# aerius-labs/paillier-halo2

Measured on AMD Instinct MI355X. Metric: Paillier-encrypt proofs/s (2048-bit n, k=17); MSM achieved HBM GB/s vs peak, higher is better.
Workload: dtype u32 limbs (29-bit reduced radix, 254-bit modular integers), u64 limbs (4096-bit integers)

## Files before the change

### paillier_halo2_amd/csrc/pz_quotient.hip

```cpp
#include "fp29.cuh"
#include "pz_internal.h"

static inline Fr fp_one_host() {
    static const uint64_t ONE[4] = {0xac96341c4ffffffbULL, 0x36fc76959f60cd29ULL, 0x666ea36f7879462eULL, 0x0e0a77c19a07df2fULL};
    Fr r;
    memcpy(r.v, ONE, 32);
    return r;
}
static inline Fr fr_from_u64(const uint64_t x[4]) {
    Fr r;
    memcpy(r.v, x, 32);
    return r;
}

typedef F29<FrTag> Fr29;
__device__ __forceinline__ Fr29 fr29_c261(const Fr& c) { return f29_to_261(f29_from_fp(c)); }
__device__ __forceinline__ Fr29 fr29_one256() {
    Fr29 r;
#pragma unroll
    for (int i = 0; i < 9; ++i) r.v[i] = P29<FrTag>::R256(i);
    return r;
}

struct S29 {
    u32 v[9];
};
static bool host_fr_canonical(const uint64_t c[4]) {
    static const uint64_t R[4] = {0x43e1f593f0000001ULL, 0x2833e84879b97091ULL, 0xb85045b68181585dULL, 0x30644e72e131a029ULL};
    for (int i = 3; i >= 0; --i)
        if (c[i] != R[i]) return c[i] < R[i];
    return false;
}
static S29 host_fr_shl(const uint64_t c[4], unsigned k) {
    static const uint64_t R[4] = {0x43e1f593f0000001ULL, 0x2833e84879b97091ULL, 0xb85045b68181585dULL, 0x30644e72e131a029ULL};
    uint64_t x[4] = {c[0], c[1], c[2], c[3]};
    for (unsigned t = 0; t < k; ++t) {
        for (int i = 3; i > 0; --i) x[i] = (x[i] << 1) | (x[i - 1] >> 63);
        x[0] <<= 1;
        bool ge = true;
        for (int i = 3; i >= 0; --i)
            if (x[i] != R[i]) { ge = x[i] > R[i]; break; }
        if (ge) {
            unsigned __int128 br = 0;
            for (int i = 0; i < 4; ++i) {
                const unsigned __int128 d = (unsigned __int128)x[i] - R[i] - br;
                x[i] = (uint64_t)d;
                br = (d >> 64) & 1;
            }
        }
    }
    S29 r;
    for (int i = 0; i < 9; ++i) {
        const unsigned bit = 29u * i, j = bit >> 6, o = bit & 63;
        uint64_t w = x[j] >> o;
        if (o > 35 && j + 1 < 4) w |= x[j + 1] << (64 - o);
        r.v[i] = (u32)(w & (i < 8 ? 0x1fffffffull : 0xffffffffull));
    }
    return r;
}
static void host_fr_mul(const uint64_t a[4], const uint64_t b[4], uint64_t out[4]) {
    static const uint64_t R[4] = {0x43e1f593f0000001ULL, 0x2833e84879b97091ULL, 0xb85045b68181585dULL, 0x30644e72e131a029ULL};
    const uint64_t INV = 0xc2e1f593efffffffULL;
    uint64_t t[6] = {0, 0, 0, 0, 0, 0};
    for (int i = 0; i < 4; ++i) {
        unsigned __int128 c = 0;
        for (int j = 0; j < 4; ++j) {
            c += (unsigned __int128)a[j] * b[i] + t[j];
            t[j] = (uint64_t)c;
            c >>= 64;
        }
        c += t[4];
        t[4] = (uint64_t)c;
        t[5] = (uint64_t)(c >> 64);
        const uint64_t m = t[0] * INV;
        c = ((unsigned __int128)m * R[0] + t[0]) >> 64;
        for (int j = 1; j < 4; ++j) {
            c += (unsigned __int128)m * R[j] + t[j];
            t[j - 1] = (uint64_t)c;
            c >>= 64;
        }
        c += t[4];
        t[3] = (uint64_t)c;
        t[4] = t[5] + (uint64_t)(c >> 64);
    }
    bool ge = t[4] != 0;
    if (!ge) {
        ge = true;
        for (int i = 3; i >= 0; --i)
            if (t[i] != R[i]) { ge = t[i] > R[i]; break; }
    }
    if (ge) {
        unsigned __int128 br = 0;
        for (int i = 0; i < 4; ++i) {
            const unsigned __int128 d = (unsigned __int128)t[i] - R[i] - br;
            t[i] = (uint64_t)d;
            br = (d >> 64) & 1;
        }
    }
    memcpy(out, t, 32);
}
static void host_fr_pow(const uint64_t a[4], unsigned e, uint64_t out[4]) {
    static const uint64_t ONE[4] = {0xac96341c4ffffffbULL, 0x36fc76959f60cd29ULL, 0x666ea36f7879462eULL, 0x0e0a77c19a07df2fULL};
    uint64_t acc[4], sq[4];
    memcpy(acc, ONE, 32);
    memcpy(sq, a, 32);
    for (; e; e >>= 1) {
        if (e & 1) host_fr_mul(acc, sq, acc);
        host_fr_mul(sq, sq, sq);
    }
    memcpy(out, acc, 32);
}
extern "C" int pzx_host_selftest(void) {
    static const uint64_t ONE[4] = {0xac96341c4ffffffbULL, 0x36fc76959f60cd29ULL, 0x666ea36f7879462eULL, 0x0e0a77c19a07df2fULL};
    auto limbs_of = [](const uint64_t x[4]) { return host_fr_shl(x, 0); };
    auto same = [](const S29& a, const S29& b) { return memcmp(a.v, b.v, sizeof a.v) == 0; };
    uint64_t two[4], acc[4], pw[4];
    {
        const S29 d = host_fr_shl(ONE, 1);
        unsigned __int128 carry = 0;
        memset(two, 0, sizeof two);
        for (int i = 0; i < 9; ++i) {
            const unsigned bit = 29u * i, j = bit >> 6, o = bit & 63;
            two[j] |= (uint64_t)d.v[i] << o;
            if (o > 35 && j + 1 < 4) two[j + 1] |= (uint64_t)d.v[i] >> (64 - o);
        }
        (void)carry;
    }
    if (!same(limbs_of(two), host_fr_shl(ONE, 1))) return 1;
    host_fr_mul(ONE, ONE, acc);
    if (memcmp(acc, ONE, 32)) return 2;
    memcpy(acc, ONE, 32);
    for (unsigned k = 1; k <= 300; ++k) {
        host_fr_mul(acc, two, acc);
        if (!same(limbs_of(acc), host_fr_shl(ONE, k))) return 100 + (int)k;
        if (k % 37 == 0 || k == 300) {
            host_fr_pow(two, k, pw);
            if (memcmp(pw, acc, 32)) return 1000 + (int)k;
        }
    }
    return 0;
}
extern "C" void pzx_host_fr_mul(const uint64_t a[4], const uint64_t b[4], uint64_t out[4]) { host_fr_mul(a, b, out); }
extern "C" void pzx_host_fr_pow(const uint64_t a[4], unsigned e, uint64_t out[4]) { host_fr_pow(a, e, out); }
extern "C" void pzx_host_fr_shl(const uint64_t c[4], unsigned k, uint32_t out[9]) {
    const S29 r = host_fr_shl(c, k);
    memcpy(out, r.v, sizeof r.v);
}
__device__ __forceinline__ Fr29 f29_add_s(const Fr29& a, const u32 (&b)[9]) {
    Fr29 r;
#pragma unroll
    for (int i = 0; i < 9; ++i) r.v[i] = a.v[i] + b[i];
    return r;
}

__global__ __launch_bounds__(256) void k_batch_invert(Fr* __restrict__ a, Fr* __restrict__ scratch, size_t n, size_t T,
                                                      unsigned K, Fr* __restrict__ mul_io) {
    const size_t t = (size_t)blockIdx.x * blockDim.x + threadIdx.x;
    if (t >= T) return;
    Fr29 acc = fr29_one256();
    for (unsigned j = 0; j < K; ++j) {
        const size_t i = t + (size_t)j * T;
        if (i >= n) break;
        const Fr v = fp_load<FrTag>(a + i);
        if (fp_is_zero(v)) continue;
        Fr w;
        f29_pack(acc, w.v);
        fp_store(scratch + i, w);
        acc = f29_mul(acc, f29_from_fp_shl5(v));
    }
    Fr29 inv = f29_mul(f29_inv(acc), fr29_one256());
    for (unsigned j = K; j-- > 0;) {
        const size_t i = t + (size_t)j * T;
        if (i >= n) continue;
        const Fr v = fp_load<FrTag>(a + i);
        if (fp_is_zero(v)) {
            if (mul_io) fp_store(mul_io + i, fp_zero<FrTag>());
            continue;
        }
        const Fr29 ai = f29_mul(inv, f29_load<FrTag>(scratch + i));
        if (mul_io) f29_store_product(mul_io + i, f29_mul(ai, f29_load_shl5<FrTag>(mul_io + i)));
        else f29_store_product(a + i, ai);
        inv = f29_mul(inv, f29_from_fp_shl5(v));
    }
}

int pz_batch_invert_internal(pz_ctx* ctx, Fr* d_a, size_t n, Fr* d_mul_io) {
    if (!n) return PZ_OK;
    void* scr;
    PZCHK(pz_ws_get(ctx, WS_BIG_A, n * 32, &scr));
    unsigned K = 8;
    while (K < 64 && n / (K * 2) >= 16384) K *= 2;
    while (K < 512 && n / (K * 2) >= 262144) K *= 2;
    const size_t T = pz_div_up(n, K);
    hipLaunchKernelGGL(k_batch_invert, dim3(pz_div_up(T, 256)), dim3(256), 0, ctx->stream, d_a, (Fr*)scr, n, T, K, d_mul_io);
    HIPCHK(ctx, hipGetLastError());
    return PZ_OK;
}

extern "C" int pz_fr_batch_invert_dev(pz_ctx* ctx, uint64_t* d_a, size_t n) {
    if (!ctx || (n && !d_a)) return PZ_ERR_INVALID;
    PZ_ENTER(ctx);
    return pz_batch_invert_internal(ctx, (Fr*)d_a, n, nullptr);
}

#define PP_K 16u
__global__ __launch_bounds__(256) void k_pp_local(const Fr* __restrict__ a, size_t as, size_t n, Fr* __restrict__ excl,
                                                  Fr* __restrict__ block_tot, unsigned nb) {
    __shared__ u32 s[9 * 256];
    a += (size_t)blockIdx.y * as;
    const size_t t = (size_t)blockIdx.x * 256 + threadIdx.x;
    const size_t lo = t * PP_K;
    Fr29 p = fr29_one256();
    for (unsigned j = 0; j < PP_K; ++j)
        if (lo + j < n) p = f29_mul(p, f29_load_shl5<FrTag>(a + lo + j));
    p = f29_to_261(p);
#pragma unroll
    for (int i = 0; i < 9; ++i) s[i * 256 + threadIdx.x] = p.v[i];
    __syncthreads();
    for (unsigned off = 1; off < 256; off <<= 1) {
        Fr29 u;
        if (threadIdx.x >= off) {
#pragma unroll
            for (int i = 0; i < 9; ++i) u.v[i] = s[i * 256 + threadIdx.x - off];
        }
        __syncthreads();
        if (threadIdx.x >= off) {
            p = f29_mul(u, p);
#pragma unroll
            for (int i = 0; i < 9; ++i) s[i * 256 + threadIdx.x] = p.v[i];
        }
        __syncthreads();
    }
    Fr29 e = f29_one<FrTag>();
    if (threadIdx.x) {
#pragma unroll
        for (int i = 0; i < 9; ++i) e.v[i] = s[i * 256 + threadIdx.x - 1];
    }
    Fr w;
    f29_pack(e, w.v);
    fp_store(excl + (size_t)blockIdx.y * nb * 256 + t, w);
    if (threadIdx.x == 255) f29_store_product(block_tot + (size_t)blockIdx.y * nb + blockIdx.x, f29_to_256(p));
}
__global__ void k_pp_blocks(Fr* __restrict__ block_tot, unsigned nb, size_t n_cols, Fr z0) {
    const size_t col = (size_t)blockIdx.x * blockDim.x + threadIdx.x;
    if (col >= n_cols) return;
    Fr* bt = block_tot + col * nb;
    Fr run = z0;
    for (unsigned b = 0; b < nb; ++b) {
        Fr t = fp_load<FrTag>(bt + b);
        fp_store(bt + b, run);
        run = fp_mul(run, t);
    }
}
__global__ __launch_bounds__(256) void k_pp_apply(const Fr* __restrict__ a, size_t as, size_t n, const Fr* __restrict__ excl,
                                                  const Fr* __restrict__ block_tot, unsigned nb, Fr* __restrict__ z, size_t zs) {
    a += (size_t)blockIdx.y * as;
    z += (size_t)blockIdx.y * zs;
    const size_t t = (size_t)blockIdx.x * 256 + threadIdx.x;
    const size_t lo = t * PP_K;
    if (lo >= n) return;
    Fr29 cur = f29_mul(f29_load<FrTag>(block_tot + (size_t)blockIdx.y * nb + blockIdx.x),
                       f29_load<FrTag>(excl + (size_t)blockIdx.y * nb * 256 + t));
    for (unsigned j = 0; j < PP_K && lo + j < n; ++j) {
        const Fr v = fp_load<FrTag>(a + lo + j);
        f29_store_product(z + lo + j, cur);
        cur = f29_mul(cur, f29_from_fp_shl5(v));
    }
}

int pz_prefix_product_batch_internal(pz_ctx* ctx, const Fr* d_a, size_t a_stride, size_t n_cols, size_t n, Fr z0, Fr* d_z,
                                     size_t z_stride) {
    if (!n || !n_cols) return PZ_OK;
    if (n_cols > 65535) return PZ_ERR_INVALID;
    const unsigned nb = pz_div_up(pz_div_up(n, PP_K), 256);
    void* ws;
    PZCHK(pz_ws_get(ctx, WS_BIG_B, n_cols * ((size_t)nb * 256 + nb) * 32, &ws));
    Fr* excl = (Fr*)ws;
    Fr* tot = excl + n_cols * (size_t)nb * 256;
    hipLaunchKernelGGL(k_pp_local, dim3(nb, (unsigned)n_cols), dim3(256), 0, ctx->stream, d_a, a_stride, n, excl, tot, nb);
    hipLaunchKernelGGL(k_pp_blocks, dim3(pz_div_up(n_cols, 64)), dim3(64), 0, ctx->stream, tot, nb, n_cols, z0);
    hipLaunchKernelGGL(k_pp_apply, dim3(nb, (unsigned)n_cols), dim3(256), 0, ctx->stream, d_a, a_stride, n, (const Fr*)excl,
                       (const Fr*)tot, nb, d_z, z_stride);
    HIPCHK(ctx, hipGetLastError());
    return PZ_OK;
}
int pz_prefix_product_internal(pz_ctx* ctx, const Fr* d_a, size_t n, Fr z0, Fr* d_z) {
    return pz_prefix_product_batch_internal(ctx, d_a, n, 1, n, z0, d_z, n);
}

extern "C" int pz_fr_prefix_product_dev(pz_ctx* ctx, const uint64_t* d_a, size_t n, const uint64_t z0[4], uint64_t* d_z) {
    if (!ctx || !z0 || (n && (!d_a || !d_z))) return PZ_ERR_INVALID;
    PZ_ENTER(ctx);
    return pz_prefix_product_internal(ctx, (const Fr*)d_a, n, fr_from_u64(z0), (Fr*)d_z);
}

__global__ __launch_bounds__(256) void k_perm_terms(const Fr* __restrict__ cols, size_t cs, const Fr* __restrict__ sigma,
                                                    size_t ss, unsigned m, size_t n, const Fr* __restrict__ wpow, Fr beta,
                                                    Fr gamma, Fr delta0, Fr delta, Fr* __restrict__ num,
                                                    Fr* __restrict__ den) {
    const size_t i = (size_t)blockIdx.x * blockDim.x + threadIdx.x;
    if (i >= n) return;
    const Fr29 g = fr29_c261(gamma), d = fr29_c261(delta), beta266 = f29_to_261(fr29_c261(beta));
    Fr29 nm = fr29_one256(), dn = nm;
    Fr29 bd = f29_mul(f29_mul(beta266, f29_from_fp(delta0)), f29_load_shl5<FrTag>(wpow + i));
    for (unsigned j = 0; j < m; ++j) {
        const Fr29 v = f29_add(f29_load_shl5<FrTag>(cols + (size_t)j * cs + i), g);
        const Fr29 sg = f29_load<FrTag>(sigma + (size_t)j * ss + i);
        nm = f29_mul(nm, f29_add(v, bd));
        dn = f29_mul(dn, f29_add(v, f29_mul(beta266, sg)));
        bd = f29_mul(bd, d);
    }
    f29_store<0>(num + i, nm);
    f29_store<0>(den + i, dn);
}

extern "C" int pz_permutation_product_dev(pz_ctx* ctx, const uint64_t* d_cols, size_t col_stride, const uint64_t* d_sigma,
                                          size_t sigma_stride, size_t m, uint32_t log_n, const uint64_t omega[4],
                                          const uint64_t beta[4], const uint64_t gamma[4], const uint64_t delta_start[4],
                                          const uint64_t delta[4], const uint64_t z0[4], uint64_t* d_z) {
    if (!ctx || !omega || !beta || !gamma || !delta_start || !delta || !z0 || !d_z || log_n > 26) return PZ_ERR_INVALID;
    if (m && (!d_cols || !d_sigma)) return PZ_ERR_INVALID;
    if (col_stride % 4 || sigma_stride % 4 || m > 65535) return PZ_ERR_INVALID;
    const size_t n = (size_t)1 << log_n;
    if (m > 1 && (col_stride < 4 * n || sigma_stride < 4 * n)) return PZ_ERR_INVALID;
    PZ_ENTER(ctx);
    void *wp, *ws;
    PZCHK(pz_get_pow_table(ctx, omega, n, &wp));
    PZCHK(pz_ws_get(ctx, WS_BIG_C, 2 * n * 32, &ws));
    Fr* num = (Fr*)ws;
    Fr* den = num + n;
    hipLaunchKernelGGL(k_perm_terms, dim3(pz_div_up(n, 256)), dim3(256), 0, ctx->stream, (const Fr*)d_cols, col_stride / 4,
                       (const Fr*)d_sigma, sigma_stride / 4, (unsigned)m, n, (const Fr*)wp, fr_from_u64(beta), fr_from_u64(gamma),
                       fr_from_u64(delta_start), fr_from_u64(delta), num, den);
    HIPCHK(ctx, hipGetLastError());
    PZCHK(pz_batch_invert_internal(ctx, den, n, num));
    return pz_prefix_product_internal(ctx, num, n, fr_from_u64(z0), (Fr*)d_z);
}

__global__ __launch_bounds__(256) void k_perm_terms_sets(const Fr* __restrict__ cols, size_t cs, const Fr* __restrict__ sigma,
                                                         size_t ss, unsigned m, unsigned chunk_len, size_t n,
                                                         const Fr* __restrict__ wpow, const Fr* __restrict__ dpow,
                                                         S29 beta266, S29 g, S29 d, Fr* __restrict__ num, Fr* __restrict__ den,
                                                         unsigned set0) {
    const size_t i = (size_t)blockIdx.x * blockDim.x + threadIdx.x;
    if (i >= n) return;
    const unsigned c0 = (set0 + blockIdx.y) * chunk_len, set = blockIdx.y;
    Fr29 nm = fr29_one256(), dn = nm;
    Fr29 bd = f29_mul(f29_mul_s(f29_load<FrTag>(dpow + c0), beta266.v), f29_load_shl5<FrTag>(wpow + i));
    Fr v_n = fp_load<FrTag>(cols + (size_t)c0 * cs + i), s_n = fp_load<FrTag>(sigma + (size_t)c0 * ss + i);
    for (unsigned c = c0; c < c0 + chunk_len && c < m; ++c) {
        const Fr29 v = f29_add_s(f29_from_fp_shl5(v_n), g.v);
        const Fr29 sg = f29_from_fp(s_n);
        const unsigned cn = (c + 1 < c0 + chunk_len && c + 1 < m) ? c + 1 : c;
        v_n = fp_load<FrTag>(cols + (size_t)cn * cs + i);
        s_n = fp_load<FrTag>(sigma + (size_t)cn * ss + i);
        nm = f29_mul(nm, f29_add(v, bd));
        dn = f29_mul(dn, f29_add(v, f29_mul_s(sg, beta266.v)));
        bd = f29_mul_s(bd, d.v);
    }
    f29_store_product(num + (size_t)set * n + i, nm);
    f29_store_product(den + (size_t)set * n + i, dn);
}
__global__ __launch_bounds__(256) void k_perm_chain(const Fr* __restrict__ z, size_t zs, unsigned n_sets, size_t u, Fr* __restrict__ mult) {
    __shared__ Fr s_p[256];
    const unsigned per = (n_sets + 255u) / 256u, lo = threadIdx.x * per, hi = lo + per < n_sets ? lo + per : n_sets;
    Fr p = fp_one<FrTag>();
    for (unsigned j = lo; j < hi; ++j) p = fp_mul(p, fp_load<FrTag>(z + (size_t)j * zs + u));
    s_p[threadIdx.x] = p;
    __syncthreads();
    for (unsigned off = 1; off < 256; off <<= 1) {
        Fr v = fp_one<FrTag>();
        if (threadIdx.x >= off) v = s_p[threadIdx.x - off];
        __syncthreads();
        if (threadIdx.x >= off) {
            p = fp_mul(v, p);
            s_p[threadIdx.x] = p;
        }
        __syncthreads();
    }
    Fr c = threadIdx.x ? s_p[threadIdx.x - 1] : fp_one<FrTag>();
    for (unsigned j = lo; j < hi; ++j) {
        fp_store(mult + j, c);
        c = fp_mul(c, fp_load<FrTag>(z + (size_t)j * zs + u));
    }
}
__global__ __launch_bounds__(256) void k_scale_sets(Fr* __restrict__ z, size_t zs, size_t n, const Fr* __restrict__ mult) {
    const size_t i = (size_t)blockIdx.x * blockDim.x + threadIdx.x;
    if (i >= n || blockIdx.y == 0) return;
    Fr* p = z + (size_t)blockIdx.y * zs + i;
    fp_store(p, fp_mul(fp_load<FrTag>(p), fp_load<FrTag>(mult + blockIdx.y)));
}

extern "C" int pz_permutation_product_sets_dev(pz_ctx* ctx, const uint64_t* d_cols, size_t col_stride, const uint64_t* d_sigma,
                                               size_t sigma_stride, size_t m, uint32_t chunk_len, uint32_t log_n,
                                               size_t usable_rows, const uint64_t omega[4], const uint64_t beta[4],
                                               const uint64_t gamma[4], const uint64_t delta[4], uint64_t* d_z,
                                               size_t z_stride) {
    if (!ctx || !d_cols || !d_sigma || !d_z || !omega || !beta || !gamma || !delta || m == 0 || chunk_len == 0 || log_n > 26)
        return PZ_ERR_INVALID;
    const size_t n = (size_t)1 << log_n;
    const size_t n_sets = (m + chunk_len - 1) / chunk_len;
    if (col_stride % 4 || sigma_stride % 4 || z_stride % 4 || usable_rows >= n || n_sets > 65535 || m > 0xffffffu) return PZ_ERR_INVALID;
    if ((m > 1 && (col_stride < 4 * n || sigma_stride < 4 * n)) || (n_sets > 1 && z_stride < 4 * n)) return PZ_ERR_INVALID;
    if (!host_fr_canonical(beta) || !host_fr_canonical(gamma) || !host_fr_canonical(delta)) return PZ_ERR_INVALID;
    PZ_ENTER(ctx);
    void *wp, *dp, *ws, *mu;
    PZCHK(pz_get_pow_table(ctx, omega, n, &wp));
    PZCHK(pz_get_pow_table(ctx, delta, m, &dp));
    size_t sb = ((size_t)4 << 30) / (2 * n * 32);
    if (sb < 1) sb = 1;
    if (sb > n_sets) sb = n_sets;
    PZCHK(pz_ws_get(ctx, WS_BIG_C, 2 * sb * n * 32, &ws));
    PZCHK(pz_ws_get(ctx, WS_MISC, n_sets * 32, &mu));
    Fr* num = (Fr*)ws;
    Fr* den = num + sb * n;
    for (size_t s0 = 0; s0 < n_sets; s0 += sb) {
        const size_t ns = n_sets - s0 < sb ? n_sets - s0 : sb;
        hipLaunchKernelGGL(k_perm_terms_sets, dim3(pz_div_up(n, 256), (unsigned)ns), dim3(256), 0, ctx->stream,
                           (const Fr*)d_cols, col_stride / 4, (const Fr*)d_sigma, sigma_stride / 4, (unsigned)m, (unsigned)chunk_len, n,
                           (const Fr*)wp, (const Fr*)dp, host_fr_shl(beta, 10), host_fr_shl(gamma, 5), host_fr_shl(delta, 5), num, den,
                           (unsigned)s0);
        HIPCHK(ctx, hipGetLastError());
        PZCHK(pz_batch_invert_internal(ctx, den, ns * n, num));
        PZCHK(pz_prefix_product_batch_internal(ctx, num, n, ns, n, fp_one_host(), (Fr*)d_z + s0 * (z_stride / 4), z_stride / 4));
    }
    if (n_sets > 1) {
        hipLaunchKernelGGL(k_perm_chain, dim3(1), dim3(256), 0, ctx->stream, (const Fr*)d_z, z_stride / 4, (unsigned)n_sets,
                           usable_rows, (Fr*)mu);
        hipLaunchKernelGGL(k_scale_sets, dim3(pz_div_up(n, 256), (unsigned)n_sets), dim3(256), 0, ctx->stream, (Fr*)d_z,
                           z_stride / 4, n, (const Fr*)mu);
        HIPCHK(ctx, hipGetLastError());
    }
    return PZ_OK;
}

__global__ __launch_bounds__(256) void k_quotient_gate(const Fr* __restrict__ adv, size_t as, const Fr* __restrict__ sel,
                                                       size_t ss, unsigned n_cols, size_t N, unsigned step, S29 y261,
                                                       Fr* __restrict__ h) {
    const size_t i = (size_t)blockIdx.x * blockDim.x + threadIdx.x;
    if (i >= N) return;
    const size_t i1 = (i + step) & (N - 1), i2 = (i + 2 * (size_t)step) & (N - 1), i3 = (i + 3 * (size_t)step) & (N - 1);
    Fr29 acc = f29_load<FrTag>(h + i);
    for (unsigned j = 0; j < n_cols; ++j) {
        const Fr* a = adv + (size_t)j * as;
        const Fr29 a0 = f29_load<FrTag>(a + i), a1 = f29_load<FrTag>(a + i1), a3 = f29_load<FrTag>(a + i3);
        const Fr29 a2 = f29_load_shl5<FrTag>(a + i2), sl = f29_load_shl5<FrTag>(sel + (size_t)j * ss + i);
        const Fr29 e = f29_sub<2, 29>(f29_add(a0, f29_mul(a1, a2)), a3);
        acc = f29_mul2_s(acc, y261.v, e, sl);
    }
    f29_store<0>(h + i, acc);
}

extern "C" int pz_quotient_gate_dev(pz_ctx* ctx, const uint64_t* d_adv_ext, size_t adv_stride, const uint64_t* d_sel_ext,
                                    size_t sel_stride, size_t n_cols, uint32_t log_ext, uint32_t rot_step,
                                    const uint64_t y[4], uint64_t* d_h) {
    if (!ctx || !y || !d_h || log_ext > 28 || (n_cols && (!d_adv_ext || !d_sel_ext))) return PZ_ERR_INVALID;
    if (adv_stride % 4 || sel_stride % 4 || n_cols > 0xffffffffu) return PZ_ERR_INVALID;
    const size_t N = (size_t)1 << log_ext;
    if (rot_step == 0 || rot_step >= N) return PZ_ERR_INVALID;
    if (n_cols > 1 && (adv_stride < 4 * N || sel_stride < 4 * N)) return PZ_ERR_INVALID;
    if (!host_fr_canonical(y)) return PZ_ERR_INVALID;
    if (n_cols == 0) return PZ_OK;
    PZ_ENTER(ctx);
    hipLaunchKernelGGL(k_quotient_gate, dim3(pz_div_up(N, 256)), dim3(256), 0, ctx->stream, (const Fr*)d_adv_ext,
                       adv_stride / 4, (const Fr*)d_sel_ext, sel_stride / 4, (unsigned)n_cols, N, (unsigned)rot_step,
                       host_fr_shl(y, 5), (Fr*)d_h);
    HIPCHK(ctx, hipGetLastError());
    return PZ_OK;
}

__global__ void k_vanishing_inv(Fr g, Fr w_ext, unsigned log_n, unsigned E, Fr* __restrict__ out) {
    const unsigned r = threadIdx.x;
    if (blockIdx.x || r >= E) return;
    Fr x = g;
    for (unsigned k = 0; k < r; ++k) x = fp_mul(x, w_ext);
    for (unsigned k = 0; k < log_n; ++k) x = fp_sqr(x);
    fp_store(out + r, fp_inv(fp_sub(x, fp_one<FrTag>())));
}
__global__ __launch_bounds__(256) void k_scale_periodic(Fr* __restrict__ h, size_t N, const Fr* __restrict__ tab,
                                                        unsigned mask) {
    const size_t i = (size_t)blockIdx.x * blockDim.x + threadIdx.x;
    if (i < N) fp_store(h + i, fp_mul(fp_load<FrTag>(h + i), fp_load<FrTag>(tab + (i & mask))));
}

extern "C" int pz_quotient_finish_dev(pz_ctx* ctx, uint64_t* d_h, uint32_t log_n, uint32_t log_e, const uint64_t coset_g[4],
                                      const uint64_t omega_ext[4]) {
    if (!ctx || !d_h || !coset_g || !omega_ext || log_e > 6 || log_n + log_e > 28) return PZ_ERR_INVALID;
    PZ_ENTER(ctx);
    const unsigned E = 1u << log_e;
    const size_t N = (size_t)1 << (log_n + log_e);
    void* tab;
    PZCHK(pz_ws_get(ctx, WS_MISC, E * 32, &tab));
    hipLaunchKernelGGL(k_vanishing_inv, dim3(1), dim3(64), 0, ctx->stream, fr_from_u64(coset_g), fr_from_u64(omega_ext),
                       (unsigned)log_n, E, (Fr*)tab);
    hipLaunchKernelGGL(k_scale_periodic, dim3(pz_div_up(N, 256)), dim3(256), 0, ctx->stream, (Fr*)d_h, N, (const Fr*)tab,
                       E - 1);
    HIPCHK(ctx, hipGetLastError());
    return PZ_OK;
}

__global__ __launch_bounds__(256) void k_mul_table_cols(Fr* __restrict__ a, size_t cs, size_t n, const Fr* __restrict__ tab) {
    const size_t i = (size_t)blockIdx.x * blockDim.x + threadIdx.x;
    if (i >= n) return;
    Fr* p = a + (size_t)blockIdx.y * cs + i;
    fp_store(p, fp_mul(fp_load<FrTag>(p), fp_load<FrTag>(tab + i)));
}

extern "C" int pz_fr_distribute_powers_dev(pz_ctx* ctx, uint64_t* d_a, size_t n_cols, size_t col_stride, size_t n,
                                           const uint64_t g[4], const uint64_t c[4]) {
    if (!ctx || !g || (n_cols && n && !d_a) || col_stride % 4 || (n_cols > 1 && col_stride < 4 * n)) return PZ_ERR_INVALID;
    if (n_cols == 0 || n == 0) return PZ_OK;
    if (n_cols > 65535) return PZ_ERR_INVALID;
    PZ_ENTER(ctx);
    void* tab;
    PZCHK(pz_get_pow_table(ctx, g, n, &tab, c));
    hipLaunchKernelGGL(k_mul_table_cols, dim3(pz_div_up(n, 256), (unsigned)n_cols), dim3(256), 0, ctx->stream, (Fr*)d_a,
                       col_stride / 4, n, (const Fr*)tab);
    HIPCHK(ctx, hipGetLastError());
    return PZ_OK;
}

#define KD_K 64u
__global__ __launch_bounds__(256) void k_kd_local(const Fr* __restrict__ a, size_t cs, size_t n, Fr x, Fr* __restrict__ L,
                                                  size_t n_chunks) {
    const size_t c = (size_t)blockIdx.x * blockDim.x + threadIdx.x;
    if (c >= n_chunks) return;
    const Fr* p = a + (size_t)blockIdx.y * cs;
    const size_t lo = c * KD_K, hi = (lo + KD_K < n ? lo + KD_K : n);
    Fr v = fp_zero<FrTag>();
    for (size_t i = hi; i-- > lo;) v = fp_add(fp_mul(v, x), fp_load<FrTag>(p + i));
    fp_store(L + (size_t)blockIdx.y * n_chunks + c, v);
}
__global__ __launch_bounds__(256) void k_kd_carry(Fr* __restrict__ L, size_t n_chunks, Fr x) {
    __shared__ Fr s_v[256], s_x[256];
    Fr* l = L + (size_t)blockIdx.x * n_chunks;
    Fr xk = x;
    for (unsigned s = 1; s < KD_K; s <<= 1) xk = fp_sqr(xk);
    const size_t per = (n_chunks + 255) / 256;
    const size_t lo = threadIdx.x * per, hi = lo + per < n_chunks ? lo + per : n_chunks;
    Fr V = fp_zero<FrTag>(), X = fp_one<FrTag>();
    for (size_t c = hi; c-- > lo && c < n_chunks;) {
        V = fp_add(fp_load<FrTag>(l + c), fp_mul(xk, V));
        X = fp_mul(X, xk);
    }
    s_v[threadIdx.x] = V;
    s_x[threadIdx.x] = X;
    __syncthreads();
    for (unsigned off = 1; off < 256; off <<= 1) {
        Fr v = s_v[threadIdx.x], xx = s_x[threadIdx.x];
        Fr uv = fp_zero<FrTag>(), ux = fp_one<FrTag>();
        const bool has = threadIdx.x + off < 256;
        if (has) { uv = s_v[threadIdx.x + off]; ux = s_x[threadIdx.x + off]; }
        __syncthreads();
        if (has) {
            s_v[threadIdx.x] = fp_add(v, fp_mul(xx, uv));
            s_x[threadIdx.x] = fp_mul(xx, ux);
        }
        __syncthreads();
    }
    Fr carry = threadIdx.x + 1 < 256 ? s_v[threadIdx.x + 1] : fp_zero<FrTag>();
    for (size_t c = hi; c-- > lo && c < n_chunks;) {
        Fr t = fp_load<FrTag>(l + c);
        fp_store(l + c, carry);
        carry = fp_add(t, fp_mul(xk, carry));
    }
}
__global__ __launch_bounds__(256) void k_kd_apply(const Fr* a, size_t cs, size_t n, Fr x,
                                                  const Fr* __restrict__ L, size_t n_chunks, Fr* q, size_t qs) {
    const size_t c = (size_t)blockIdx.x * blockDim.x + threadIdx.x;
    if (c >= n_chunks) return;
    const Fr* p = a + (size_t)blockIdx.y * cs;
    Fr* o = q + (size_t)blockIdx.y * qs;
    const size_t lo = c * KD_K, hi = (lo + KD_K < n ? lo + KD_K : n);
    Fr cur = fp_load<FrTag>(L + (size_t)blockIdx.y * n_chunks + c);
    for (size_t i = hi; i-- > lo;) {
        Fr ai = fp_load<FrTag>(p + i);
        fp_store(o + i, cur);
        cur = fp_add(ai, fp_mul(x, cur));
    }
}

extern "C" int pz_poly_div_linear_dev(pz_ctx* ctx, const uint64_t* d_coeffs, size_t n_cols, size_t col_stride, size_t n,
                                      const uint64_t x[4], uint64_t* d_q, size_t q_stride) {
    if (!ctx || !x || (n_cols && n && (!d_coeffs || !d_q)) || col_stride % 4 || q_stride % 4) return PZ_ERR_INVALID;
    if (n_cols > 1 && (col_stride < 4 * n || q_stride < 4 * n)) return PZ_ERR_INVALID;
    if (n_cols == 0 || n == 0) return PZ_OK;
    if (n_cols > 65535) return PZ_ERR_INVALID;
    PZ_ENTER(ctx);
    const size_t nch = pz_div_up(n, KD_K);
    void* L;
    PZCHK(pz_ws_get(ctx, WS_BIG_A, n_cols * nch * 32, &L));
    Fr xv = fr_from_u64(x);
    hipLaunchKernelGGL(k_kd_local, dim3(pz_div_up(nch, 256), (unsigned)n_cols), dim3(256), 0, ctx->stream,
                       (const Fr*)d_coeffs, col_stride / 4, n, xv, (Fr*)L, nch);
    hipLaunchKernelGGL(k_kd_carry, dim3((unsigned)n_cols), dim3(256), 0, ctx->stream, (Fr*)L, nch, xv);
    hipLaunchKernelGGL(k_kd_apply, dim3(pz_div_up(nch, 256), (unsigned)n_cols), dim3(256), 0, ctx->stream,
                       (const Fr*)d_coeffs, col_stride / 4, n, xv, (const Fr*)L, nch, (Fr*)d_q, q_stride / 4);
    HIPCHK(ctx, hipGetLastError());
    return PZ_OK;
}

struct PermQ {
    const Fr *cols, *sigma, *z, *l0, *llast, *lactive, *xpow;
    size_t cs, ss, zs, N;
    unsigned n_sets, chunk_len, m_total, step, last_rot;
    unsigned set_lo, n_sets_total, head;
    S29 y, gamma, delta, beta266;
    S29 bx266;
    S29 y_chain, y_sets;
    S29 y_sets_d;
};
template <bool SPLIT> __global__ __launch_bounds__(256) void k_quotient_permutation(PermQ q, Fr* __restrict__ h, Fr* __restrict__ hd) {
    const size_t i0 = (size_t)blockIdx.x * blockDim.x + threadIdx.x;
    const size_t half = q.N >> 1;
    if (i0 >= half) return;
    const size_t mask = q.N - 1;
    size_t row[2], i_next[2], i_last[2];
    Fr29 acc[2];
#pragma unroll
    for (int r = 0; r < 2; ++r) {
        row[r] = i0 + (r ? half : 0);
        i_next[r] = (row[r] + q.step) & mask;
        i_last[r] = (row[r] + q.N - (size_t)q.last_rot * q.step) & mask;
        acc[r] = f29_load<FrTag>(h + row[r]);
    }
#pragma unroll
    for (int r = 0; r < 2 && q.head; ++r) {
        const size_t i = row[r];
        const Fr29 one = fr29_one256();
        const Fr29 l0 = f29_load_shl5<FrTag>(q.l0 + i);
        const Fr29 z_first = f29_load<FrTag>(q.z + i);
        acc[r] = f29_mul2_s(acc[r], q.y.v, f29_sub<2, 29>(one, z_first), l0);
        {
            const Fr29 ll = f29_load_shl5<FrTag>(q.llast + i);
            const Fr zl = fp_load<FrTag>(q.z + (size_t)(q.n_sets_total - 1) * q.zs + i);
            const Fr29 z_lastset = f29_from_fp(zl);
            acc[r] = f29_mul2_s(acc[r], q.y.v, f29_sub<2, 29>(f29_mul(z_lastset, f29_from_fp_shl5(zl)), z_lastset), ll);
        }
        if (q.n_sets_total > 1) {
            Fr29 t0 = f29_sub<2, 29>(f29_load<FrTag>(q.z + q.zs + i), f29_load<FrTag>(q.z + i_last[r]));
            for (unsigned j = 2; j < q.n_sets_total; ++j) {
                const Fr29 d = f29_sub<2, 29>(f29_load<FrTag>(q.z + (size_t)j * q.zs + i), f29_load<FrTag>(q.z + (size_t)(j - 1) * q.zs + i_last[r]));
                t0 = f29_add(f29_mul_s(t0, q.y.v), d);
            }
            acc[r] = f29_mul2_s(acc[r], q.y_chain.v, t0, l0);
        }
    }
    Fr29 cur = f29_mul_s(f29_load<FrTag>(q.xpow + i0), q.bx266.v);
    unsigned c = 0;
    Fr v_n[2], s_n[2];
#pragma unroll
    for (int r = 0; r < 2; ++r) {
        v_n[r] = fp_load<FrTag>(q.cols + row[r]);
        s_n[r] = fp_load<FrTag>(q.sigma + row[r]);
    }
    Fr29 hs[2];
    for (unsigned j = 0; j < q.n_sets; ++j) {
        Fr29 left[2], right[2];
#pragma unroll
        for (int r = 0; r < 2; ++r) {
            left[r] = f29_load<FrTag>(q.z + (size_t)(q.set_lo + j) * q.zs + i_next[r]);
            right[r] = f29_load<FrTag>(q.z + (size_t)(q.set_lo + j) * q.zs + row[r]);
        }
        for (unsigned t = 0; t < q.chunk_len && c < q.m_total; ++t, ++c) {
            const unsigned cn = c + 1 < q.m_total ? c + 1 : c;
#pragma unroll
            for (int r = 0; r < 2; ++r) {
                const Fr29 v = f29_add_s(f29_from_fp_shl5(v_n[r]), q.gamma.v);
                const Fr29 sg = f29_from_fp(s_n[r]);
                v_n[r] = fp_load<FrTag>(q.cols + (size_t)cn * q.cs + row[r]);
                s_n[r] = fp_load<FrTag>(q.sigma + (size_t)cn * q.ss + row[r]);
                left[r] = f29_mul(left[r], f29_add(v, f29_mul_s(sg, q.beta266.v)));
                right[r] = f29_mul(right[r], r ? f29_sub<2, 29>(v, cur) : f29_add(v, cur));
            }
            cur = f29_mul_s(cur, q.delta.v);
        }
#pragma unroll
        for (int r = 0; r < 2; ++r) {
            const Fr29 diff = f29_sub<2, 29>(left[r], right[r]);
            hs[r] = j ? f29_add(f29_mul_s(hs[r], q.y.v), diff) : diff;
        }
    }
#pragma unroll
    for (int r = 0; r < 2; ++r) {
        if (SPLIT) {
            f29_store<0>(hd + row[r], f29_mul2_s(f29_load<FrTag>(hd + row[r]), q.y_sets_d.v, hs[r], f29_one<FrTag>()));
            acc[r] = f29_mul_s(acc[r], q.y_sets.v);
        } else {
            acc[r] = f29_mul2_s(acc[r], q.y_sets.v, hs[r], f29_load_shl5<FrTag>(q.lactive + row[r]));
        }
        f29_store<0>(h + row[r], acc[r]);
    }
}

static int quotient_permutation_launch(pz_ctx* ctx, const uint64_t* d_cols_ext, size_t col_stride, const uint64_t* d_sigma_ext,
                                       size_t sigma_stride, const uint64_t* d_z_ext, size_t z_stride, uint32_t n_sets_total,
                                       uint32_t set_lo, uint32_t n_sets, uint32_t chunk_len, uint32_t m_cols, int head, uint32_t log_ext,
                                       uint32_t rot_step, uint32_t last_rotation, const uint64_t* d_l0, const uint64_t* d_l_last,
                                       const uint64_t* d_l_active, const uint64_t beta[4], const uint64_t gamma[4],
                                       const uint64_t delta[4], const uint64_t coset_g[4], const uint64_t omega_ext[4],
                                       const uint64_t y[4], uint64_t* d_h, uint64_t* d_hd) {
    if (!ctx || !d_cols_ext || !d_sigma_ext || !d_z_ext || !d_l0 || !d_l_last || (!d_l_active && !d_hd) || !beta || !gamma || !delta ||
        !coset_g || !omega_ext || !y || !d_h || d_h == d_hd)
        return PZ_ERR_INVALID;
    if (log_ext > 28 || log_ext == 0 || n_sets == 0 || chunk_len == 0 || m_cols == 0 || col_stride % 4 || sigma_stride % 4 || z_stride % 4)
        return PZ_ERR_INVALID;
    if (n_sets_total == 0 || (size_t)set_lo + n_sets > n_sets_total) return PZ_ERR_INVALID;
    const size_t N = (size_t)1 << log_ext;
    if ((size_t)n_sets * chunk_len < m_cols || (size_t)(n_sets - 1) * chunk_len >= m_cols) return PZ_ERR_INVALID;
    if (set_lo + n_sets < n_sets_total && (size_t)n_sets * chunk_len != m_cols) return PZ_ERR_INVALID;
    if (rot_step == 0 || rot_step >= N || (size_t)last_rotation * rot_step >= N) return PZ_ERR_INVALID;
    if ((m_cols > 1 && (col_stride < 4 * N || sigma_stride < 4 * N)) || (n_sets_total > 1 && z_stride < 4 * N)) return PZ_ERR_INVALID;
    if (!host_fr_canonical(beta) || !host_fr_canonical(gamma) || !host_fr_canonical(delta) || !host_fr_canonical(y)) return PZ_ERR_INVALID;
    PZ_ENTER(ctx);
    PermQ q;
    q.cols = (const Fr*)d_cols_ext; q.sigma = (const Fr*)d_sigma_ext; q.z = (const Fr*)d_z_ext;
    q.l0 = (const Fr*)d_l0; q.llast = (const Fr*)d_l_last; q.lactive = (const Fr*)d_l_active;
    q.cs = col_stride / 4; q.ss = sigma_stride / 4; q.zs = z_stride / 4; q.N = N;
    q.n_sets = n_sets; q.chunk_len = chunk_len; q.m_total = m_cols; q.step = rot_step; q.last_rot = last_rotation;
    q.set_lo = set_lo; q.n_sets_total = n_sets_total; q.head = head ? 1u : 0u;
    q.beta266 = host_fr_shl(beta, 10); q.gamma = host_fr_shl(gamma, 5); q.delta = host_fr_shl(delta, 5); q.y = host_fr_shl(y, 5);
    uint64_t yp[4], bx[4];
    host_fr_pow(delta, set_lo * chunk_len, bx);
    host_fr_mul(bx, beta, bx);
    q.bx266 = host_fr_shl(bx, 10);
    host_fr_pow(y, n_sets_total - 1, yp);
    q.y_chain = host_fr_shl(yp, 5);
    host_fr_pow(y, n_sets, yp);
    q.y_sets = host_fr_shl(yp, 5);
    host_fr_pow(y, n_sets + (head ? 2 + (n_sets_total > 1 ? n_sets_total - 1 : 0) : 0), yp);
    q.y_sets_d = host_fr_shl(yp, 5);
    void* xp;
    PZCHK(pz_get_pow_table(ctx, omega_ext, N, &xp, coset_g));
    q.xpow = (const Fr*)xp;
    if (d_hd) hipLaunchKernelGGL(k_quotient_permutation<true>, dim3(pz_div_up(N / 2, 256)), dim3(256), 0, ctx->stream, q, (Fr*)d_h, (Fr*)d_hd);
    else hipLaunchKernelGGL(k_quotient_permutation<false>, dim3(pz_div_up(N / 2, 256)), dim3(256), 0, ctx->stream, q, (Fr*)d_h, (Fr*)nullptr);
// ... 262 lines not shown
```

Before: 1.427.

## Fold permutation set chaining into prefix-product block totals

Removes the separate k_perm_chain and k_scale_sets passes, which rescaled every z column after all sets were computed. A new chain kernel computes each set's value at usable_rows from the local scan results, carries the cross-set product across batches, and folds the multiplier into the block totals before k_pp_apply. This avoids a full read-modify-write of the z grand-product columns, at the cost of two small extra launches per batch, one of them a single-block kernel. It also adds a bounded-memory entry point that takes term_bytes as a parameter.

After: 1.433, median of 6. Within noise of the previous version (+0.5%).

```diff
diff --git a/paillier_halo2_amd/csrc/pz_quotient.hip b/paillier_halo2_amd/csrc/pz_quotient.hip
--- a/paillier_halo2_amd/csrc/pz_quotient.hip
+++ b/paillier_halo2_amd/csrc/pz_quotient.hip
@@ -268,8 +268,54 @@
     }
 }
 
-int pz_prefix_product_batch_internal(pz_ctx* ctx, const Fr* d_a, size_t a_stride, size_t n_cols, size_t n, Fr z0, Fr* d_z,
-                                     size_t z_stride) {
+__global__ __launch_bounds__(256) void k_pp_chain(const Fr* __restrict__ a, size_t as, const Fr* __restrict__ excl,
+                                                  const Fr* __restrict__ block_tot, unsigned nb, unsigned n_cols, size_t u,
+                                                  Fr* __restrict__ carry, int first, Fr* __restrict__ mult) {
+    __shared__ Fr s_p[256];
+    const unsigned per = (n_cols + 255u) / 256u, lo = threadIdx.x * per, hi = lo + per < n_cols ? lo + per : n_cols;
+    const size_t ut = u / PP_K;
+    const Fr c0 = first ? fp_one<FrTag>() : fp_load<FrTag>(carry);
+    Fr p = fp_one<FrTag>();
+    for (unsigned j = lo; j < hi; ++j) {
+        Fr29 cur = f29_mul(f29_load<FrTag>(block_tot + (size_t)j * nb + ut / 256), f29_load<FrTag>(excl + (size_t)j * nb * 256 + ut));
+        for (size_t i = ut * PP_K; i < u; ++i) cur = f29_mul(cur, f29_load_shl5<FrTag>(a + (size_t)j * as + i));
+        f29_store_product(mult + j, cur);
+        p = fp_mul(p, fp_load<FrTag>(mult + j));
+    }
+    s_p[threadIdx.x] = p;
+    __syncthreads();
+    for (unsigned off = 1; off < 256; off <<= 1) {
+        Fr v = fp_one<FrTag>();
+        if (threadIdx.x >= off) v = s_p[threadIdx.x - off];
+        __syncthreads();
+        if (threadIdx.x >= off) {
+            p = fp_mul(v, p);
+            s_p[threadIdx.x] = p;
+        }
+        __syncthreads();
+    }
+    Fr c = threadIdx.x ? fp_mul(c0, s_p[threadIdx.x - 1]) : c0;
+    for (unsigned j = lo; j < hi; ++j) {
+        const Fr zu = fp_load<FrTag>(mult + j);
+        fp_store(mult + j, c);
+        c = fp_mul(c, zu);
+    }
+    if (threadIdx.x == 255) fp_store(carry, fp_mul(c0, p));
+}
+__global__ __launch_bounds__(256) void k_pp_scale_blocks(Fr* __restrict__ block_tot, unsigned nb, size_t n_cols, const Fr* __restrict__ mult) {
+    const size_t i = (size_t)blockIdx.x * blockDim.x + threadIdx.x;
+    if (i >= n_cols * nb) return;
+    fp_store(block_tot + i, fp_mul(fp_load<FrTag>(block_tot + i), fp_load<FrTag>(mult + i / nb)));
+}
+
+struct PpChain {
+    size_t u;
+    Fr* carry;
+    Fr* mult;
+    int first;
+};
+static int pp_batch(pz_ctx* ctx, const Fr* d_a, size_t a_stride, size_t n_cols, size_t n, Fr z0, Fr* d_z, size_t z_stride,
+                    const PpChain* chain) {
     if (!n || !n_cols) return PZ_OK;
     if (n_cols > 65535) return PZ_ERR_INVALID;
     const unsigned nb = pz_div_up(pz_div_up(n, PP_K), 256);
@@ -279,10 +325,20 @@
     Fr* tot = excl + n_cols * (size_t)nb * 256;
     hipLaunchKernelGGL(k_pp_local, dim3(nb, (unsigned)n_cols), dim3(256), 0, ctx->stream, d_a, a_stride, n, excl, tot, nb);
     hipLaunchKernelGGL(k_pp_blocks, dim3(pz_div_up(n_cols, 64)), dim3(64), 0, ctx->stream, tot, nb, n_cols, z0);
+    if (chain) {
+        hipLaunchKernelGGL(k_pp_chain, dim3(1), dim3(256), 0, ctx->stream, d_a, a_stride, (const Fr*)excl, (const Fr*)tot, nb,
+                           (unsigned)n_cols, chain->u, chain->carry, chain->first, chain->mult);
+        hipLaunchKernelGGL(k_pp_scale_blocks, dim3(pz_div_up(n_cols * nb, 256)), dim3(256), 0, ctx->stream, tot, nb, n_cols,
+                           (const Fr*)chain->mult);
+    }
     hipLaunchKernelGGL(k_pp_apply, dim3(nb, (unsigned)n_cols), dim3(256), 0, ctx->stream, d_a, a_stride, n, (const Fr*)excl,
                        (const Fr*)tot, nb, d_z, z_stride);
     HIPCHK(ctx, hipGetLastError());
     return PZ_OK;
+}
+int pz_prefix_product_batch_internal(pz_ctx* ctx, const Fr* d_a, size_t a_stride, size_t n_cols, size_t n, Fr z0, Fr* d_z,
+                                     size_t z_stride) {
+    return pp_batch(ctx, d_a, a_stride, n_cols, n, z0, d_z, z_stride, nullptr);
 }
 int pz_prefix_product_internal(pz_ctx* ctx, const Fr* d_a, size_t n, Fr z0, Fr* d_z) {
     return pz_prefix_product_batch_internal(ctx, d_a, n, 1, n, z0, d_z, n);
@@ -361,41 +417,10 @@
     f29_store_product(num + (size_t)set * n + i, nm);
     f29_store_product(den + (size_t)set * n + i, dn);
 }
-__global__ __launch_bounds__(256) void k_perm_chain(const Fr* __restrict__ z, size_t zs, unsigned n_sets, size_t u, Fr* __restrict__ mult) {
-    __shared__ Fr s_p[256];
-    const unsigned per = (n_sets + 255u) / 256u, lo = threadIdx.x * per, hi = lo + per < n_sets ? lo + per : n_sets;
-    Fr p = fp_one<FrTag>();
-    for (unsigned j = lo; j < hi; ++j) p = fp_mul(p, fp_load<FrTag>(z + (size_t)j * zs + u));
-    s_p[threadIdx.x] = p;
-    __syncthreads();
-    for (unsigned off = 1; off < 256; off <<= 1) {
-        Fr v = fp_one<FrTag>();
-        if (threadIdx.x >= off) v = s_p[threadIdx.x - off];
-        __syncthreads();
-        if (threadIdx.x >= off) {
-            p = fp_mul(v, p);
-            s_p[threadIdx.x] = p;
-        }
-        __syncthreads();
-    }
-    Fr c = threadIdx.x ? s_p[threadIdx.x - 1] : fp_one<FrTag>();
-    for (unsigned j = lo; j < hi; ++j) {
-        fp_store(mult + j, c);
-        c = fp_mul(c, fp_load<FrTag>(z + (size_t)j * zs + u));
-    }
-}
-__global__ __launch_bounds__(256) void k_scale_sets(Fr* __restrict__ z, size_t zs, size_t n, const Fr* __restrict__ mult) {
-    const size_t i = (size_t)blockIdx.x * blockDim.x + threadIdx.x;
-    if (i >= n || blockIdx.y == 0) return;
-    Fr* p = z + (size_t)blockIdx.y * zs + i;
-    fp_store(p, fp_mul(fp_load<FrTag>(p), fp_load<FrTag>(mult + blockIdx.y)));
-}
-
-extern "C" int pz_permutation_product_sets_dev(pz_ctx* ctx, const uint64_t* d_cols, size_t col_stride, const uint64_t* d_sigma,
-                                               size_t sigma_stride, size_t m, uint32_t chunk_len, uint32_t log_n,
-                                               size_t usable_rows, const uint64_t omega[4], const uint64_t beta[4],
-                                               const uint64_t gamma[4], const uint64_t delta[4], uint64_t* d_z,
-                                               size_t z_stride) {
+static int permutation_product_sets(pz_ctx* ctx, const uint64_t* d_cols, size_t col_stride, const uint64_t* d_sigma,
+                                    size_t sigma_stride, size_t m, uint32_t chunk_len, uint32_t log_n, size_t usable_rows,
+                                    const uint64_t omega[4], const uint64_t beta[4], const uint64_t gamma[4],
+                                    const uint64_t delta[4], uint64_t* d_z, size_t z_stride, size_t term_bytes) {
     if (!ctx || !d_cols || !d_sigma || !d_z || !omega || !beta || !gamma || !delta || m == 0 || chunk_len == 0 || log_n > 26)
         return PZ_ERR_INVALID;
     const size_t n = (size_t)1 << log_n;
@@ -407,11 +432,11 @@
     void *wp, *dp, *ws, *mu;
     PZCHK(pz_get_pow_table(ctx, omega, n, &wp));
     PZCHK(pz_get_pow_table(ctx, delta, m, &dp));
-    size_t sb = ((size_t)4 << 30) / (2 * n * 32);
+    size_t sb = term_bytes / (2 * n * 32);
     if (sb < 1) sb = 1;
     if (sb > n_sets) sb = n_sets;
     PZCHK(pz_ws_get(ctx, WS_BIG_C, 2 * sb * n * 32, &ws));
-    PZCHK(pz_ws_get(ctx, WS_MISC, n_sets * 32, &mu));
+    PZCHK(pz_ws_get(ctx, WS_MISC, (sb + 1) * 32, &mu));
     Fr* num = (Fr*)ws;
     Fr* den = num + sb * n;
     for (size_t s0 = 0; s0 < n_sets; s0 += sb) {
@@ -422,16 +447,26 @@
                            (unsigned)s0);
         HIPCHK(ctx, hipGetLastError());
         PZCHK(pz_batch_invert_internal(ctx, den, ns * n, num));
-        PZCHK(pz_prefix_product_batch_internal(ctx, num, n, ns, n, fp_one_host(), (Fr*)d_z + s0 * (z_stride / 4), z_stride / 4));
-    }
-    if (n_sets > 1) {
-        hipLaunchKernelGGL(k_perm_chain, dim3(1), dim3(256), 0, ctx->stream, (const Fr*)d_z, z_stride / 4, (unsigned)n_sets,
-                           usable_rows, (Fr*)mu);
-        hipLaunchKernelGGL(k_scale_sets, dim3(pz_div_up(n, 256), (unsigned)n_sets), dim3(256), 0, ctx->stream, (Fr*)d_z,
-                           z_stride / 4, n, (const Fr*)mu);
-        HIPCHK(ctx, hipGetLastError());
-    }
-    return PZ_OK;
+        const PpChain chain = {usable_rows, (Fr*)mu + sb, (Fr*)mu, s0 == 0};
+        PZCHK(pp_batch(ctx, num, n, ns, n, fp_one_host(), (Fr*)d_z + s0 * (z_stride / 4), z_stride / 4, n_sets > 1 ? &chain : nullptr));
+    }
+    return PZ_OK;
+}
+extern "C" int pz_permutation_product_sets_dev(pz_ctx* ctx, const uint64_t* d_cols, size_t col_stride, const uint64_t* d_sigma,
+                                               size_t sigma_stride, size_t m, uint32_t chunk_len, uint32_t log_n,
+                                               size_t usable_rows, const uint64_t omega[4], const uint64_t beta[4],
+                                               const uint64_t gamma[4], const uint64_t delta[4], uint64_t* d_z,
+                                               size_t z_stride) {
+    return permutation_product_sets(ctx, d_cols, col_stride, d_sigma, sigma_stride, m, chunk_len, log_n, usable_rows, omega, beta, gamma,
+                                    delta, d_z, z_stride, (size_t)4 << 30);
+}
+extern "C" int pzx_permutation_product_sets_bounded(pz_ctx* ctx, const uint64_t* d_cols, size_t col_stride, const uint64_t* d_sigma,
+                                                    size_t sigma_stride, size_t m, uint32_t chunk_len, uint32_t log_n,
+                                                    size_t usable_rows, const uint64_t omega[4], const uint64_t beta[4],
+                                                    const uint64_t gamma[4], const uint64_t delta[4], uint64_t* d_z,
+                                                    size_t z_stride, size_t term_bytes) {
+    return permutation_product_sets(ctx, d_cols, col_stride, d_sigma, sigma_stride, m, chunk_len, log_n, usable_rows, omega, beta, gamma,
+                                    delta, d_z, z_stride, term_bytes);
 }
 
 __global__ __launch_bounds__(256) void k_quotient_gate(const Fr* __restrict__ adv, size_t as, const Fr* __restrict__ sel,
```
